# manhofer/Line3Dpp

Hardware: NVIDIA B200
Metric: matched_line_pairs_per_sec (higher is better)
Workload: dtype f32

## Files before the change

line3dpp_b200/csrc/l3d_match.cu:

```cuda
#include "l3d_match.cuh"
#include "l3d_device_f64.cuh"

__global__ void __launch_bounds__(256) k_prep_segments(const float4* __restrict__ segs, const L3DViewDev* __restrict__ views,
                                                       int num_views, long long total, float4* __restrict__ cache)
{
    long long idx = (long long)blockIdx.x * blockDim.x + threadIdx.x;
    if (idx >= total) return;
    int lo = 0, hi = num_views - 1;
    while (lo < hi) {
        int mid = (lo + hi + 1) >> 1;
        if (views[mid].seg_off <= idx) lo = mid; else hi = mid - 1;
    }
    const L3DViewDev* v = views + lo;
    float4 s = segs[idx];
    float3 r1 = normalize3(mulmat_h(v->RtKinv, s.x, s.y));
    float3 r2 = normalize3(mulmat_h(v->RtKinv, s.z, s.w));
    float3 n = normalize3(cross3(r1, r2));
    cache[3 * idx] = make_float4(r1.x, r1.y, r1.z, r2.x);
    cache[3 * idx + 1] = make_float4(r2.y, r2.z, n.x, n.y);
    cache[3 * idx + 2] = make_float4(n.z, 0.f, 0.f, 0.f);
}

__global__ void __launch_bounds__(256) k_prep_segments_f64(const float4* __restrict__ segs, const L3DViewDev* __restrict__ views,
                                                           int num_views, long long total, double* __restrict__ cache)
{
    long long idx = (long long)blockIdx.x * blockDim.x + threadIdx.x;
    if (idx >= total) return;
    int lo = 0, hi = num_views - 1;
    while (lo < hi) {
        int mid = (lo + hi + 1) >> 1;
        if (views[mid].seg_off <= idx) lo = mid; else hi = mid - 1;
    }
    const L3DViewDev* v = views + lo;
    float4 s = segs[idx];
    D3 r1 = dray(v->RtKinv_d, (double)s.x, (double)s.y), r2 = dray(v->RtKinv_d, (double)s.z, (double)s.w);
    D3 n = dnormalized(dcross(r1, r2));
    double* o = cache + 9 * idx;
    o[0] = r1.x; o[1] = r1.y; o[2] = r1.z; o[3] = r2.x; o[4] = r2.y; o[5] = r2.z; o[6] = n.x; o[7] = n.y; o[8] = n.z;
}

struct MatchSmem {
    uint4 stage[MK_STAGES][MK_TT];
    uint2 rowK[MK_ROWS];
    int cls_off[L3D_ARC_NCLS + 2];
    unsigned char rowall[MK_ROWS];
    unsigned long long lists[MK_ROWS][MK_CAP + 1];
    float4 rowA[MK_ROWS];
    float4 rowB[MK_ROWS];
    float row_thr[MK_ROWS];
    int list_cnt[MK_ROWS];
    unsigned int queue[MK_WARPS][128];
    unsigned int queue2[MK_WARPS][96];
    unsigned long long bars[MK_STAGES];
    const float4* tsegs; const float4* cache;
    long long src_base, toff;
    float3 Cs, Ct;
    float epi; int knn, Nt;
    int cap;
    const double* cache_d; const float4* ssegs;
    double Fd[9]; D3 Csd, Ctd;
    long long R0; l3d_match_rec* recs_out;
};
size_t l3d_match_smem_bytes() { return sizeof(MatchSmem); }

__device__ __forceinline__ int rank_in_row(const unsigned long long* list, int n, unsigned long long k)
{
    int r = 0;
    for (int j = 0; j < n; ++j) r += list[j] > k;
    return r;
}

__device__ __noinline__ void prune_row(MatchSmem& S, int row, int lane)
{
    const int knn = S.knn; const float epi = S.epi;
    __syncwarp();
    const int n = min(S.list_cnt[row], S.cap);
    const unsigned long long k = lane < n ? S.lists[row][lane] : 0ull;
    int r;
    if (knn <= 16) {
        bool active = lane < n;
        const unsigned int hi = (unsigned int)(k >> 32), lo = (unsigned int)k;
        r = 64;
        const int rounds = min(knn, n);
        for (int i = 0; i < rounds; ++i) {
            const unsigned int m = __reduce_max_sync(0xffffffffu, active ? hi : 0u);
            bool c = active && hi == m;
            unsigned int bm = __ballot_sync(0xffffffffu, c);
            if (__popc(bm) > 1) { const unsigned int l = __reduce_max_sync(0xffffffffu, c ? lo : 0u); c = c && lo == l; }
            if (c) { r = i; active = false; }
        }
    } else r = rank_in_row(S.lists[row], n, k);
    __syncwarp();
    if (lane < n && r < knn) S.lists[row][r] = k;
    __syncwarp();
    if (lane == 0) {
        S.list_cnt[row] = min(n, knn);
        if (n >= knn) {
            const float kth = key_overlap(S.lists[row][knn - 1]);
            S.row_thr[row] = kth;
            S.rowB[row].w = 0.95f * fmaxf(kth, epi);
        }
    }
    __syncwarp();
}

__device__ __noinline__ bool eval_candidate_f64(const MatchSmem& S, int rl, unsigned int j, float* ov_out, float* dep)
{
    const float4 sp = __ldg(S.ssegs + rl);
    const D3 e1 = dmulmat(S.Fd, d3((double)sp.x, (double)sp.y, 1.0)), e2 = dmulmat(S.Fd, d3((double)sp.z, (double)sp.w, 1.0));
    bool valid;
    const float ov = exact_overlap_f64(__ldg(S.tsegs + j), e1, e2, &valid);
    if (!(valid && ov > S.epi && ov >= S.row_thr[rl])) return false;
    const SegRaysD s = load_rays_d(S.cache_d, S.src_base + rl), t = load_rays_d(S.cache_d, S.toff + j);
    double d[4];
    exact_depths_f64(s, t, S.Csd, S.Ctd, d);
    if (!(d[0] > L3D_EPS_D && d[1] > L3D_EPS_D && d[2] > L3D_EPS_D && d[3] > L3D_EPS_D)) return false;
    *ov_out = ov;
    dep[0] = (float)d[0]; dep[1] = (float)d[1]; dep[2] = (float)d[2]; dep[3] = (float)d[3];
    return true;
}

template <int MODE, int KEEP>
__device__ __noinline__ void exact_batch(MatchSmem& S, unsigned int entry, bool has, int lane)
{
    const float4* __restrict__ tsegs = S.tsegs; const float4* __restrict__ cache = S.cache;
    const long long src_base = S.src_base, toff = S.toff;
    const float3 Cs = S.Cs, Ct = S.Ct;
    const float epi = S.epi; const int knn = S.knn;
    bool pending = false;
    unsigned long long key = 0ull;
    int rl = 0;
    if (has) {
        rl = (int)(entry >> 24);
        unsigned int j = entry & 0xFFFFFFu;
        if (j >= (unsigned int)S.Nt) j = 0u, has = false;
        float ov = 0.0f, d[4];
        bool ok = false;
        if (MODE) { if (has) ok = eval_candidate_f64(S, rl, j, &ov, d); }
        else {
            float4 q = __ldg(tsegs + j);
            float4 rA = S.rowA[rl], rB = S.rowB[rl];
            bool inv;
            ov = exact_overlap(q, make_float3(rA.x, rA.y, rA.z), make_float3(rA.w, rB.x, rB.y), &inv);
            if (has && ov > epi && ov >= S.row_thr[rl]) {
                SegRays s = load_rays(cache, src_base + rl), t = load_rays(cache, toff + j);
                exact_depths(s, t, Cs, Ct, d);
                ok = d[0] > 0.0f && d[1] > 0.0f && d[2] > 0.0f && d[3] > 0.0f;
            }
        }
        if (ok) {
            if (KEEP == 0) { key = make_key(ov, j); pending = true; }
            else {
                const int slot = atomicAdd(&S.list_cnt[rl], 1);
                if (KEEP == 2 && slot < knn) {
                    l3d_match_rec rec;
                    rec.tgt_seg = j; rec.overlap = ov; rec.d_p1 = d[0]; rec.d_p2 = d[1]; rec.d_q1 = d[2]; rec.d_q2 = d[3];
                    S.recs_out[(S.R0 + rl) * knn + slot] = rec;
                }
            }
        }
    }
    while (KEEP == 0) {
        if (pending) {
            int slot = atomicAdd(&S.list_cnt[rl], 1);
            if (slot < S.cap) { S.lists[rl][slot] = key; pending = false; }
        }
        unsigned int pm = __ballot_sync(0xffffffffu, pending);
        if (!pm) break;
        unsigned int todo = pm;
        while (todo) {
            int leader = __ffs(todo) - 1;
            int row = __shfl_sync(0xffffffffu, rl, leader);
            prune_row(S, row, lane);
            unsigned int mine = __ballot_sync(0xffffffffu, pending && rl == row);
            todo &= ~mine;
            if (knn >= S.cap) {
                while (mine) {
                    int l = __ffs(mine) - 1;
                    mine &= mine - 1;
                    unsigned long long k = __shfl_sync(0xffffffffu, key, l);
                    if (lane == 0 && k > S.lists[row][S.cap - 1]) S.lists[row][S.cap - 1] = k;
                    if (lane == l) pending = false;
                    prune_row(S, row, lane);
                }
            }
        }
    }
    __syncwarp();
}

template <int MODE, int KEEP>
__device__ __noinline__ void finalize_rows(MatchSmem& S, int warp, int lane, int nrows, long long R0, int* __restrict__ counts_out,
                                           l3d_match_rec* __restrict__ recs_out)
{
    const int knn = S.knn;
    for (int r = 0; r < MK_RPW; ++r) {
        const int rl = warp * MK_RPW + r;
        if (rl >= nrows) break;
        const long long R = R0 + rl;
        if (KEEP != 0) { if (lane == 0) counts_out[R] = S.list_cnt[rl]; continue; }
        const int n = min(S.list_cnt[rl], S.cap);
        if (lane == 0) counts_out[R] = min(n, knn);
        if (n == 0) continue;
        const unsigned long long key = lane < n ? S.lists[rl][lane] : 0ull;
        const int rank = rank_in_row(S.lists[rl], n, key);
        if (lane < n && rank < knn) {
            unsigned int j = key_tgt(key);
            float d[4];
            if (MODE) {
                const SegRaysD s = load_rays_d(S.cache_d, S.src_base + rl), t = load_rays_d(S.cache_d, S.toff + j);
                double dd[4];
                exact_depths_f64(s, t, S.Csd, S.Ctd, dd);
                d[0] = (float)dd[0]; d[1] = (float)dd[1]; d[2] = (float)dd[2]; d[3] = (float)dd[3];
            } else {
                SegRays s = load_rays(S.cache, S.src_base + rl), t = load_rays(S.cache, S.toff + j);
                exact_depths(s, t, S.Cs, S.Ct, d);
            }
            l3d_match_rec rec;
            rec.tgt_seg = j; rec.overlap = key_overlap(key);
            rec.d_p1 = d[0]; rec.d_p2 = d[1]; rec.d_q1 = d[2]; rec.d_q2 = d[3];
            recs_out[R * knn + rank] = rec;
        }
    }
}

__device__ void pair_basis(const float* F, L3DPairBasis* B)
{
    double c[3][3];
    for (int k = 0; k < 3; ++k) {
        const double x = F[k], y = F[3 + k], z = F[6 + k], n = sqrt(x * x + y * y + z * z);
        c[k][0] = n > 0.0 ? x / n : 0.0; c[k][1] = n > 0.0 ? y / n : 0.0; c[k][2] = n > 0.0 ? z / n : 0.0;
    }
    double E[3] = {0.0, 0.0, 0.0}, best = 0.0;
    for (int a = 0; a < 3; ++a)
        for (int b = a + 1; b < 3; ++b) {
            const double x = c[a][1] * c[b][2] - c[a][2] * c[b][1], y = c[a][2] * c[b][0] - c[a][0] * c[b][2], z = c[a][0] * c[b][1] - c[a][1] * c[b][0];
            const double n = x * x + y * y + z * z;
            if (n > best) { best = n; E[0] = x; E[1] = y; E[2] = z; }
        }
    const double nan = __longlong_as_double(0x7ff8000000000000ll);
    double n[3] = {E[0] / L3D_ARC_SCALE, E[1] / L3D_ARC_SCALE, E[2]};
    const double len = sqrt(n[0] * n[0] + n[1] * n[1] + n[2] * n[2]);
    if (!(best > 1e-20) || !(len > 0.0) || !isfinite(len)) { for (int i = 0; i < 3; ++i) B->u[i] = B->v[i] = nan; return; }
    for (int i = 0; i < 3; ++i) n[i] /= len;
    int ax = 0;
    if (fabs(n[1]) < fabs(n[ax])) ax = 1;
    if (fabs(n[2]) < fabs(n[ax])) ax = 2;
    double a[3] = {0.0, 0.0, 0.0}; a[ax] = 1.0;
    double u[3] = {n[1] * a[2] - n[2] * a[1], n[2] * a[0] - n[0] * a[2], n[0] * a[1] - n[1] * a[0]};
    const double ul = sqrt(u[0] * u[0] + u[1] * u[1] + u[2] * u[2]);
    for (int i = 0; i < 3; ++i) u[i] /= ul;
    const double v[3] = {n[1] * u[2] - n[2] * u[1], n[2] * u[0] - n[0] * u[2], n[0] * u[1] - n[1] * u[0]};
    for (int i = 0; i < 3; ++i) { B->u[i] = u[i]; B->v[i] = v[i]; }
}

__device__ uint4 target_arc(const L3DPairBasis& B, float4 q, double ext, bool enabled)
{
    const uint4 none = make_uint4(0u, 0xFFFFFFFFu, 0u, 0u);
    if (!enabled) return none;
    const double x1 = (double)q.x / L3D_ARC_SCALE, y1 = (double)q.y / L3D_ARC_SCALE, x2 = (double)q.z / L3D_ARC_SCALE, y2 = (double)q.w / L3D_ARC_SCALE;
    const double a1 = x1 * B.u[0] + y1 * B.u[1] + B.u[2], b1 = x1 * B.v[0] + y1 * B.v[1] + B.v[2];
    const double dx = x2 - x1, dy = y2 - y1, ac = dx * B.u[0] + dy * B.u[1], bc = dx * B.v[0] + dy * B.v[1];
    const double len = sqrt(dx * dx + dy * dy), rhoc = sqrt(ac * ac + bc * bc);
    const double delta = (0.05 + 4e-3 * len * L3D_ARC_SCALE) / L3D_ARC_SCALE;
    if (!(len > 1e-9) || !isfinite(rhoc) || !(rhoc > 1e-3 * len) || !(ext >= 0.0)) return none;
    {
        const double lx = y1 - y2, ly = x2 - x1, lz = x1 * y2 - y1 * x2;
        const double nx = B.u[1] * B.v[2] - B.u[2] * B.v[1], ny = B.u[2] * B.v[0] - B.u[0] * B.v[2], nz = B.u[0] * B.v[1] - B.u[1] * B.v[0];
        if (!(fabs(lx * nx + ly * ny + lz * nz) > 1e-4 * sqrt(lx * lx + ly * ly + lz * lz))) return none;
    }
    const double to_units = 4294967296.0 / 3.14159265358979323846;
    const unsigned int kc = arc_units(atan2(ac, -bc));
    const double ts[4] = {-ext, 0.0, 1.0, 1.0 + ext};
    double al[4], mg[4];
    for (int i = 0; i < 4; ++i) {
        const double a = a1 + ts[i] * ac, b = b1 + ts[i] * bc, rho = sqrt(a * a + b * b);
        if (!isfinite(rho) || !(delta < 0.25 * rho)) return none;
        al[i] = (double)(unsigned int)(arc_units(atan2(a, -b)) - kc);
        mg[i] = (1.2 * delta / rho + 4e-6) * to_units;
    }
    const bool up = al[0] <= al[1] && al[1] <= al[2] && al[2] <= al[3], down = al[0] >= al[1] && al[1] >= al[2] && al[2] >= al[3];
    if (!up && !down) return none;
    const int i0 = up ? 0 : 3, i1 = up ? 1 : 2, i2 = up ? 2 : 1, i3 = up ? 3 : 0;
    const double top = 4294967295.0;
    double lo = fmax(al[i1] - mg[i1], 0.0), hi = fmin(al[i2] + mg[i2], top);
    double lox = fmin(fmax(al[i0] - mg[i0], 0.0), lo), hix = fmax(fmin(al[i3] + mg[i3], top), hi);
    lo = floor(lo); lox = floor(lox); hi = ceil(hi); hix = ceil(hix);
    if (!(hix - lox < 2147483648.0 - 524288.0)) return none;
    return make_uint4(kc + (unsigned int)lo, (unsigned int)(hi - lo), (unsigned int)(lo - lox), (unsigned int)(hix - hi));
}

__global__ void __launch_bounds__(256)
k_pair_arcs(const float4* __restrict__ segs, const L3DViewDev* __restrict__ views, const L3DPairDev* __restrict__ pairs, int first_pair,
            int enabled, double ext, uint4* __restrict__ raw, unsigned long long* __restrict__ keys, unsigned int* __restrict__ vals,
            L3DPairBasis* __restrict__ basis)
{
    __shared__ L3DPairBasis B;
    __shared__ int cnt[L3D_ARC_NCLS + 1];
    const L3DPairDev* P = pairs + first_pair + blockIdx.x;
    if (threadIdx.x == 0) pair_basis(P->F, &B);
    if (threadIdx.x <= L3D_ARC_NCLS) cnt[threadIdx.x] = 0;
    __syncthreads();
    const L3DViewDev* vt = views + P->tgt;
    const float4* t = segs + vt->seg_off;
    const int Nt = vt->nseg;
    for (int j = threadIdx.x; j < Nt; j += 256) {
        const uint4 r = target_arc(B, t[j], ext, enabled != 0);
        const int c = arc_class(r.y);
        raw[P->arc_off + j] = r;
        keys[P->arc_off + j] = ((unsigned long long)blockIdx.x << 36) | ((unsigned long long)c << 32) | (c == L3D_ARC_NCLS ? (unsigned long long)j : (unsigned long long)r.x);
        vals[P->arc_off + j] = (unsigned int)(P->arc_off + j);
        atomicAdd(&cnt[c], 1);
    }
    __syncthreads();
    if (threadIdx.x == 0) {
        int off = 0;
        for (int c = 0; c <= L3D_ARC_NCLS; ++c) { B.cls_off[c] = off; off += cnt[c]; }
        B.cls_off[L3D_ARC_NCLS + 1] = off;
        basis[first_pair + blockIdx.x] = B;
    }
}

__global__ void __launch_bounds__(256)
k_arcs_gather(long long n, const unsigned long long* __restrict__ keys, const unsigned int* __restrict__ vals, const uint4* __restrict__ raw,
              const L3DPairDev* __restrict__ pairs, int first_pair, uint4* __restrict__ out)
{
    const long long i = (long long)blockIdx.x * blockDim.x + threadIdx.x;
    if (i >= n) return;
    const unsigned long long k = keys[i];
    const unsigned int src = vals[i];
    const uint4 r = raw[src];
    const bool wide = ((k >> 32) & 0xFull) == (unsigned long long)L3D_ARC_NCLS;
    const unsigned int j = src - (unsigned int)pairs[first_pair + (int)(k >> 36)].arc_off;
    const unsigned int w16 = (r.y + 65535u) >> 16, e1 = (r.z + 65535u) >> 16, eh = (r.w + 65535u) >> 16;
    out[i] = wide ? make_uint4(0u, 0u, L3D_ARC_WIDE, j) : make_uint4(r.x, e1 | (w16 << 16), eh, j);
}

template <int MODE, int KEEP>
__device__ __forceinline__ void filter_batch(MatchSmem& S, unsigned int e0, bool has0, unsigned int e1, bool has1, int warp, int lane,
                                             unsigned int lt_mask, int& qn2)
{
    float4 q0 = make_float4(0.f, 0.f, 0.f, 0.f), q1 = q0;
    if (has0) q0 = __ldg(S.tsegs + (e0 & 0xFFFFFFu));
    if (has1) q1 = __ldg(S.tsegs + (e1 & 0xFFFFFFu));
    bool p0 = false, p1 = false;
    if (has0) { const int rl = (int)(e0 >> 24); p0 = filter_may_survive(q0, S.rowA[rl], S.rowB[rl]); }
    if (has1) { const int rl = (int)(e1 >> 24); p1 = filter_may_survive(q1, S.rowA[rl], S.rowB[rl]); }
    const unsigned int b0 = __ballot_sync(0xffffffffu, p0), b1 = __ballot_sync(0xffffffffu, p1);
    if (b0 | b1) {
        if (p0) S.queue2[warp][qn2 + __popc(b0 & lt_mask)] = e0;
        qn2 += __popc(b0);
        if (p1) S.queue2[warp][qn2 + __popc(b1 & lt_mask)] = e1;
        qn2 += __popc(b1);
        __syncwarp();
        while (qn2 >= 32) { qn2 -= 32; exact_batch<MODE, KEEP>(S, S.queue2[warp][qn2 + lane], true, lane); }
    }
}

template <int MODE, int KEEP>
__device__ __forceinline__ void match_topk_body(const float4* __restrict__ segs, const float4* __restrict__ cache, const L3DViewDev* __restrict__ views,
             const L3DPairDev* __restrict__ pairs, const int2* __restrict__ tiles, int knn, float epi,
             int* __restrict__ counts_out, l3d_match_rec* __restrict__ recs_out, const double* __restrict__ cache_d,
             const uint4* __restrict__ arcs, const L3DPairBasis* __restrict__ basis)
{
    extern __shared__ __align__(128) unsigned char smem_raw[];
    MatchSmem& S = *reinterpret_cast<MatchSmem*>(smem_raw);
    const int tid = threadIdx.x, lane = tid & 31, warp = tid >> 5;
    const int2 tile = tiles[blockIdx.x];
    const L3DPairDev* P = pairs + tile.x;
    const int row0 = tile.y;
    const L3DViewDev* vs = views + P->src;
    const L3DViewDev* vt = views + P->tgt;
    const long long soff = vs->seg_off, toff = vt->seg_off;
    const int Ns = vs->nseg, Nt = vt->nseg;
    const int nrows = min(MK_ROWS, Ns - row0);
    const float4* tsegs = segs + toff;
    const uint4* tarcs = arcs + P->arc_off;
    const int RES = MK_STAGES * MK_TT;
    const int npass = (Nt + RES - 1) / RES;
    if (tid == 0) {
        S.tsegs = tsegs; S.cache = cache; S.src_base = soff + row0; S.toff = toff; S.epi = epi; S.knn = knn; S.Nt = Nt; S.cap = MK_CAP;
        S.Cs = make_float3(vs->C[0], vs->C[1], vs->C[2]); S.Ct = make_float3(vt->C[0], vt->C[1], vt->C[2]);
        S.cache_d = cache_d; S.ssegs = segs + soff + row0; S.R0 = P->row_off + row0; S.recs_out = recs_out;
        if (MODE) {
            for (int i = 0; i < 9; ++i) S.Fd[i] = P->Fd[i];
            S.Csd = d3(vs->C_d[0], vs->C_d[1], vs->C_d[2]); S.Ctd = d3(vt->C_d[0], vt->C_d[1], vt->C_d[2]);
        }
        for (int i = 0; i < MK_STAGES; ++i) mbar_init(&S.bars[i], 1);
        mbar_fence_init();
        for (int i = 0; i < MK_STAGES && i * MK_TT < Nt; ++i) {
            const unsigned int bytes = (unsigned int)min(MK_TT, Nt - i * MK_TT) * 16u;
            mbar_expect_tx(&S.bars[i], bytes);
            tma_load_1d(S.stage[i], tarcs + (size_t)i * MK_TT, bytes, &S.bars[i]);
        }
    }
    if (tid >= MK_THREADS - (L3D_ARC_NCLS + 2)) S.cls_off[MK_THREADS - 1 - tid] = basis[tile.x].cls_off[MK_THREADS - 1 - tid];
    if (tid < MK_ROWS) {
        S.list_cnt[tid] = 0;
        S.row_thr[tid] = 0.0f;
        if (tid < nrows) {
            float4 s = __ldg(segs + soff + row0 + tid);
            float3 e1 = mulmat_h(P->F, s.x, s.y), e2 = mulmat_h(P->F, s.z, s.w);
            float g = L3D_FILTER_C1 * fmaxf(sqrtf(e1.x * e1.x + e1.y * e1.y), sqrtf(e2.x * e2.x + e2.y * e2.y));
            S.rowA[tid] = make_float4(e1.x, e1.y, e1.z, e2.x);
            S.rowB[tid] = make_float4(e2.y, e2.z, g, 0.95f * epi);
            const L3DPairBasis B = basis[tile.x];
            bool off1, off2;
            S.rowK[tid] = make_uint2(line_kappa(B, e1, &off1), line_kappa(B, e2, &off2));
            S.rowall[tid] = (off1 || off2) ? 1 : 0;
        }
    }
    __syncthreads();

    const unsigned int lt_mask = (1u << lane) - 1u;
    const uint4* ent = &S.stage[0][0];
    const int my_rows = min(MK_RPW, nrows - warp * MK_RPW);
    int qn = 0, qn2 = 0;

    for (int pass = 0; pass < npass; ++pass) {
        const int base = pass * RES, cnt = min(RES, Nt - base);
        if (pass > 0) {
            __syncthreads();
            if (tid == 0)
                for (int i = 0; i < MK_STAGES && i * MK_TT < cnt; ++i) {
                    const unsigned int bytes = (unsigned int)min(MK_TT, cnt - i * MK_TT) * 16u;
                    mbar_expect_tx(&S.bars[i], bytes);
                    tma_load_1d(S.stage[i], tarcs + (size_t)base + (size_t)i * MK_TT, bytes, &S.bars[i]);
                }
        }
        for (int i = 0; i < MK_STAGES && i * MK_TT < cnt; ++i) mbar_wait(&S.bars[i], (unsigned int)(pass & 1));
        for (int r = 0; r < my_rows; ++r) {
            const int rl = warp * MK_RPW + r;
            const uint2 kr = S.rowK[rl];
            const bool rall = S.rowall[rl] != 0;
            const bool fwd = (kr.y - kr.x) < 0x80000000u;
            const unsigned int ka = fwd ? kr.x : kr.y, kb = fwd ? kr.y : kr.x;
            int res = 0;
            {
                const int c = min(lane >> 1, L3D_ARC_NCLS - 1);
                int lo = min(max(S.cls_off[c] - base, 0), cnt), hi = min(max(S.cls_off[c + 1] - base, 0), cnt);
                const bool upper = lane & 1;
                const unsigned int key = upper ? kb + 1u : ka - (1u << (L3D_ARC_CLS0 + c));
                if (lane >= 2 * L3D_ARC_NCLS || rall) hi = lo;
                else if (upper && kb == 0xFFFFFFFFu) lo = hi;
                while (lo < hi) {
                    const int mid = (lo + hi) >> 1;
                    if (ent[mid].x < key) lo = mid + 1; else hi = mid;
                }
                res = lo;
            }
            int plo = 0, phi = 0;
            {
                const int c = min(lane >> 1, L3D_ARC_NCLS - 1);
                const int i0 = __shfl_sync(0xffffffffu, res, 2 * c), i1 = __shfl_sync(0xffffffffu, res, 2 * c + 1);
                const int s_c = min(max(S.cls_off[c] - base, 0), cnt), e_c = min(max(S.cls_off[c + 1] - base, 0), cnt);
                const bool wrap = ka - (1u << (L3D_ARC_CLS0 + c)) > kb;
                if (lane < 2 * L3D_ARC_NCLS) {
                    if (!(lane & 1)) { plo = wrap ? s_c : i0; phi = i1; }
                    else if (wrap) { plo = i0; phi = e_c; }
                } else if (lane == 2 * L3D_ARC_NCLS) { plo = min(max(S.cls_off[L3D_ARC_NCLS] - base, 0), cnt); phi = cnt; }
                if (rall) { plo = 0; phi = lane == 0 ? cnt : 0; }
            }
            unsigned int pieces = __ballot_sync(0xffffffffu, phi > plo);
            while (pieces) {
                const int p = __ffs(pieces) - 1;
                pieces &= pieces - 1u;
                const int lo = __shfl_sync(0xffffffffu, plo, p), hi = __shfl_sync(0xffffffffu, phi, p);
                for (int j0 = lo; j0 < hi; j0 += 64) {
                    const int ia = j0 + lane, ib = ia + 32;
                    bool pa = false, pb = false;
                    unsigned int ta = 0u, tb = 0u;
                    if (ia < hi) { const uint4 e = ent[ia]; pa = arc_may_match(e, kr.x, kr.y) || rall; ta = e.w; }
                    if (ib < hi) { const uint4 e = ent[ib]; pb = arc_may_match(e, kr.x, kr.y) || rall; tb = e.w; }
                    const unsigned int ba = __ballot_sync(0xffffffffu, pa), bb = __ballot_sync(0xffffffffu, pb);
                    if (ba | bb) {
                        if (pa) S.queue[warp][qn + __popc(ba & lt_mask)] = ((unsigned int)rl << 24) | ta;
                        qn += __popc(ba);
                        if (pb) S.queue[warp][qn + __popc(bb & lt_mask)] = ((unsigned int)rl << 24) | tb;
                        qn += __popc(bb);
                        __syncwarp();
                        if (qn >= 64) {
                            qn -= 64;
                            filter_batch<MODE, KEEP>(S, S.queue[warp][qn + lane], true, S.queue[warp][qn + 32 + lane], true, warp, lane, lt_mask, qn2);
                        }
                    }
                }
            }
        }
    }
    if (qn > 0) {
        const bool h0 = lane < qn, h1 = lane + 32 < qn;
        filter_batch<MODE, KEEP>(S, h0 ? S.queue[warp][lane] : 0u, h0, h1 ? S.queue[warp][lane + 32] : 0u, h1, warp, lane, lt_mask, qn2);
    }
    __syncwarp();
    if (qn2 > 0) {
        const bool has = lane < qn2;
        exact_batch<MODE, KEEP>(S, has ? S.queue2[warp][lane] : 0u, has, lane);
    }
    __syncwarp();

    finalize_rows<MODE, KEEP>(S, warp, lane, nrows, P->row_off + row0, counts_out, recs_out);
}

__global__ void __launch_bounds__(MK_THREADS, MK_MINB)
k_match_topk(const float4* __restrict__ segs, const float4* __restrict__ cache, const L3DViewDev* __restrict__ views,
             const L3DPairDev* __restrict__ pairs, const int2* __restrict__ tiles, int knn, float epi,
             int* __restrict__ counts_out, l3d_match_rec* __restrict__ recs_out, const uint4* __restrict__ arcs, const L3DPairBasis* __restrict__ basis)
{ match_topk_body<0, 0>(segs, cache, views, pairs, tiles, knn, epi, counts_out, recs_out, nullptr, arcs, basis); }

__global__ void __launch_bounds__(MK_THREADS, MK_MINB)
k_match_topk_f64(const float4* __restrict__ segs, const float4* __restrict__ cache, const L3DViewDev* __restrict__ views,
                 const L3DPairDev* __restrict__ pairs, const int2* __restrict__ tiles, int knn, float epi,
                 int* __restrict__ counts_out, l3d_match_rec* __restrict__ recs_out, const double* __restrict__ cache_d,
                 const uint4* __restrict__ arcs, const L3DPairBasis* __restrict__ basis)
{ match_topk_body<1, 0>(segs, cache, views, pairs, tiles, knn, epi, counts_out, recs_out, cache_d, arcs, basis); }

__global__ void __launch_bounds__(MK_THREADS, MK_MINB)
k_match_all(const float4* __restrict__ segs, const float4* __restrict__ cache, const L3DViewDev* __restrict__ views,
            const L3DPairDev* __restrict__ pairs, const int2* __restrict__ tiles, int stride, float epi,
            int* __restrict__ counts_out, l3d_match_rec* __restrict__ recs_out, const double* __restrict__ cache_d,
            const uint4* __restrict__ arcs, const L3DPairBasis* __restrict__ basis)
{
    if (cache_d) {
        if (stride == 0) match_topk_body<1, 1>(segs, cache, views, pairs, tiles, 0, epi, counts_out, recs_out, cache_d, arcs, basis);
        else match_topk_body<1, 2>(segs, cache, views, pairs, tiles, stride, epi, counts_out, recs_out, cache_d, arcs, basis);
    } else {
        if (stride == 0) match_topk_body<0, 1>(segs, cache, views, pairs, tiles, 0, epi, counts_out, recs_out, nullptr, arcs, basis);
        else match_topk_body<0, 2>(segs, cache, views, pairs, tiles, stride, epi, counts_out, recs_out, nullptr, arcs, basis);
    }
}

__global__ void __launch_bounds__(128) k_sort_rows(int* __restrict__ counts, l3d_match_rec* __restrict__ recs, int stride, long long rows, int topk)
{
    extern __shared__ __align__(16) unsigned char sort_smem[];
    const int warp = threadIdx.x >> 5, lane = threadIdx.x & 31, wpb = blockDim.x >> 5;
    l3d_match_rec* buf = reinterpret_cast<l3d_match_rec*>(sort_smem) + (size_t)warp * stride;
    for (long long row = (long long)blockIdx.x * wpb + warp; row < rows; row += (long long)gridDim.x * wpb) {
        const int n = min(counts[row], stride);
        if (n > 1) {
            l3d_match_rec* g = recs + row * stride;
            for (int i = lane; i < n; i += 32) buf[i] = g[i];
            __syncwarp();
            for (int i = lane; i < n; i += 32) {
                const unsigned int t = buf[i].tgt_seg;
                const float ov = buf[i].overlap;
                int r = 0;
                if (topk > 0) { for (int j = 0; j < n; ++j) r += (buf[j].overlap > ov || (buf[j].overlap == ov && buf[j].tgt_seg < t)) ? 1 : 0; if (r < topk) g[r] = buf[i]; }
                else { for (int j = 0; j < n; ++j) r += buf[j].tgt_seg < t; g[r] = buf[i]; }
            }
        }
        if (topk > 0 && lane == 0 && n > topk) counts[row] = topk;
        __syncwarp();
    }
}

struct DenseSmem {
    float4 rowA[DK_ROWS], rowB[DK_ROWS];
    float4 sray[DK_ROWS][3];
    float4 tq[DK_WARPS][32 * DK_T];
    unsigned int queue[DK_WARPS][64];
    float4* depths; float* overlaps;
    const float4* tcache;
    float3 Cs, Ct;
    float epi; int Nt, row0;
};
size_t l3d_dense_smem_bytes() { return sizeof(DenseSmem); }
int l3d_dense_rows_per_cta(int Ns, int Nt, int num_sms)
{
    const long long slots = (long long)DK_MINB * (num_sms > 0 ? num_sms : 148);
    const long long colb = (Nt + DK_WARPS * DK_T * 32 - 1) / (DK_WARPS * DK_T * 32);
    int best = 16; double best_eff = -1.0;
    for (int R = 8; R <= DK_ROWS; ++R) {
        const long long tiles = colb * ((Ns + R - 1) / R);
        const long long waves = (tiles + slots - 1) / slots;
        const double eff = (double)tiles / (double)(waves * slots);
        if (eff > best_eff + 1e-9 || (eff > best_eff - 1e-9 && R > best)) { best_eff = eff; best = R; }
    }
    return best;
}

__device__ __forceinline__ SegRays rays_from_smem(const float4* p)
{
    const float4 a = p[0], b = p[1], c = p[2];
    SegRays s;
    s.r1 = make_float3(a.x, a.y, a.z); s.r2 = make_float3(a.w, b.x, b.y); s.n = make_float3(b.z, b.w, c.x);
    return s;
}

__device__ __noinline__ void dense_exact_batch(DenseSmem& S, unsigned int entry, bool has, int warp, int x0)
{
    if (!has) return;
    const int r = (int)(entry >> 24), x = (int)(entry & 0xFFFFFFu), col = x - x0;
    const float4 q = S.tq[warp][col];
    const float4 rA = S.rowA[r], rB = S.rowB[r];
    float4 res = make_float4(-1.f, -1.f, -1.f, -1.f);
    bool inv;
    const float ov = exact_overlap(q, make_float3(rA.x, rA.y, rA.z), make_float3(rA.w, rB.x, rB.y), &inv);
    if (ov > S.epi) {
        const SegRays s = rays_from_smem(S.sray[r]), t = load_rays(S.tcache, x);
        float d[4];
        exact_depths(s, t, S.Cs, S.Ct, d);
        res = make_float4(d[0], d[1], d[2], d[3]);
    }
    const size_t o = (size_t)(S.row0 + r) * S.Nt + x;
    __stcs(S.depths + o, res);
    __stcs(S.overlaps + o, ov);
}

__device__ __forceinline__ void dense_tile(const float4* __restrict__ ssegs, int Ns, const float4* __restrict__ tsegs, int Nt,
                                           const float4* __restrict__ scache, const float4* __restrict__ tcache, const L3DMat3& F, float3 Cs, float3 Ct,
                                           float epi, float4* __restrict__ depths, float* __restrict__ overlaps, int rows_per_cta, int bx, int by)
{
    extern __shared__ __align__(128) unsigned char dense_smem_raw[];
    DenseSmem& S = *reinterpret_cast<DenseSmem*>(dense_smem_raw);
    const int tid = threadIdx.x, lane = tid & 31, warp = tid >> 5;
    const int row0 = by * rows_per_cta;
    const int nrows = min(rows_per_cta, Ns - row0);
    if (tid == 0) { S.depths = depths; S.overlaps = overlaps; S.tcache = tcache; S.Cs = Cs; S.Ct = Ct; S.epi = epi; S.Nt = Nt; S.row0 = row0; }
    if (tid < nrows) {
        float4 s = __ldg(ssegs + row0 + tid);
        float3 e1 = mulmat_h(F.m, s.x, s.y), e2 = mulmat_h(F.m, s.z, s.w);
        float g = L3D_FILTER_C1 * fmaxf(sqrtf(e1.x * e1.x + e1.y * e1.y), sqrtf(e2.x * e2.x + e2.y * e2.y));
        S.rowA[tid] = make_float4(e1.x, e1.y, e1.z, e2.x);
        S.rowB[tid] = make_float4(e2.y, e2.z, g, 0.f);
    }
    if (tid < 3 * nrows) S.sray[tid / 3][tid % 3] = __ldg(scache + 3 * (size_t)row0 + tid);
    const int x0 = (bx * DK_WARPS + warp) * (32 * DK_T);
    float4 q[DK_T];
    bool ok[DK_T];
#pragma unroll
    for (int t = 0; t < DK_T; ++t) {
        const int x = x0 + t * 32 + lane;
        ok[t] = x < Nt;
        q[t] = __ldg(tsegs + (ok[t] ? x : 0));
        S.tq[warp][t * 32 + lane] = q[t];
    }
    __syncthreads();
    if (x0 >= Nt) return;
    const unsigned int lt_mask = (1u << lane) - 1u;
    const float4 none = make_float4(-1.f, -1.f, -1.f, -1.f);
    int qn = 0;
    for (int r = 0; r < nrows; ++r) {
        const float4 rA = S.rowA[r], rB = S.rowB[r];
        const size_t orow = (size_t)(row0 + r) * Nt;
        bool pass[DK_T];
#pragma unroll
        for (int t = 0; t < DK_T; ++t) pass[t] = ok[t] && filter_may_survive(q[t], rA, rB);
#pragma unroll
        for (int t = 0; t < DK_T; ++t) {
            const int x = x0 + t * 32 + lane;
            if (ok[t] && !pass[t]) { __stcs(depths + orow + x, none); __stcs(overlaps + orow + x, 0.0f); }
            const unsigned int b = __ballot_sync(0xffffffffu, pass[t]);
            if (b) {
                if (pass[t]) S.queue[warp][qn + __popc(b & lt_mask)] = ((unsigned int)r << 24) | (unsigned int)x;
                qn += __popc(b);
                __syncwarp();
                if (qn >= 32) { qn -= 32; dense_exact_batch(S, S.queue[warp][qn + lane], true, warp, x0); }
            }
        }
    }
    if (qn > 0) dense_exact_batch(S, lane < qn ? S.queue[warp][lane] : 0u, lane < qn, warp, x0);
}

__global__ void __launch_bounds__(DK_THREADS, DK_MINB)
k_match_dense(const float4* __restrict__ ssegs, int Ns, const float4* __restrict__ tsegs, int Nt,
              const float4* __restrict__ scache, const float4* __restrict__ tcache, L3DMat3 F, float3 Cs, float3 Ct,
              float epi, float4* __restrict__ depths, float* __restrict__ overlaps, int rows_per_cta)
{ dense_tile(ssegs, Ns, tsegs, Nt, scache, tcache, F, Cs, Ct, epi, depths, overlaps, rows_per_cta, blockIdx.x, blockIdx.y); }

__global__ void __launch_bounds__(DK_THREADS, DK_MINB)
k_match_dense_batch(const L3DDenseJob* __restrict__ jobs, int njobs, float epi)
{
    __shared__ int job_s;
    if (threadIdx.x == 0) {
        int lo = 0, hi = njobs - 1;
        while (lo < hi) { const int mid = (lo + hi + 1) >> 1; if (jobs[mid].tile0 <= (long long)blockIdx.x) lo = mid; else hi = mid - 1; }
        job_s = lo;
    }
    __syncthreads();
    const L3DDenseJob& J = jobs[job_s];
    const int t = (int)((long long)blockIdx.x - J.tile0);
    dense_tile(J.ssegs, J.Ns, J.tsegs, J.Nt, J.scache, J.tcache, J.F, J.Cs, J.Ct, epi, J.depths, J.overlaps, J.rows_per_cta, t % J.colb, t / J.colb);
}

__global__ void __launch_bounds__(DK_THREADS)
k_match_dense_nofilter(const float4* __restrict__ ssegs, int Ns, const float4* __restrict__ tsegs, int Nt,
                       const float4* __restrict__ scache, const float4* __restrict__ tcache, L3DMat3 F, float3 Cs,
                       float3 Ct, float epi, float4* __restrict__ depths, float* __restrict__ overlaps)
{
    const int x = blockIdx.x * DK_THREADS + threadIdx.x;
    const int row0 = blockIdx.y * DKN_ROWS;
    const int nrows = min(DKN_ROWS, Ns - row0);
    if (x >= Nt) return;
    const float4 q = __ldg(tsegs + x);
    for (int r = 0; r < nrows; ++r) {
        float4 s4 = __ldg(ssegs + row0 + r);
        float3 e1 = mulmat_h(F.m, s4.x, s4.y), e2 = mulmat_h(F.m, s4.z, s4.w);
        float4 res = make_float4(-1.f, -1.f, -1.f, -1.f);
        bool inv;
        float ov = exact_overlap(q, e1, e2, &inv);
        if (ov > epi) {
            SegRays s = load_rays(scache, row0 + r), t = load_rays(tcache, x);
            float d[4];
            exact_depths(s, t, Cs, Ct, d);
            res = make_float4(d[0], d[1], d[2], d[3]);
        }
        const size_t o = (size_t)(row0 + r) * Nt + x;
        depths[o] = res;
        overlaps[o] = ov;
    }
}

__global__ void __launch_bounds__(256) k_compact_matches(const int* __restrict__ counts, const long long* __restrict__ row_ptr,
                                                         const l3d_match_rec* __restrict__ recs, int knn, long long rows,
                                                         l3d_match_rec* __restrict__ out)
{
    long long i = (long long)blockIdx.x * blockDim.x + threadIdx.x;
    long long row = i / knn;
    int slot = (int)(i - row * knn);
    if (row >= rows) return;
    if (slot < counts[row]) out[row_ptr[row] + slot] = recs[row * knn + slot];
}

__global__ void __launch_bounds__(256) k_fp32_peak(float* __restrict__ out, int iters, float a, float b)
{
    float x[16];
#pragma unroll
    for (int i = 0; i < 16; ++i) x[i] = (float)(threadIdx.x + i);
    for (int it = 0; it < iters; ++it) {
#pragma unroll
        for (int i = 0; i < 16; ++i) x[i] = __fmaf_rn(x[i], a, b);
    }
    float s = 0.f;
#pragma unroll
    for (int i = 0; i < 16; ++i) s += x[i];
    if (s == 123.456f) out[0] = s;
}
```

line3dpp_b200/csrc/l3d_match.cuh:

```cuda
#pragma once
#include "l3d_device.cuh"
#include "../../include/l3d_capi.h"

#ifndef MK_WARPS
#define MK_WARPS 8
#endif
#define MK_THREADS (32 * MK_WARPS)
#ifndef MK_RPW
#define MK_RPW 8
#endif
#define MK_ROWS (MK_WARPS * MK_RPW)
#ifndef MK_TT
#define MK_TT 1024
#endif
#ifndef MK_STAGES
#define MK_STAGES 3
#endif
#ifndef MK_CAP
#define MK_CAP 32
#endif
#ifndef MK_MINB
#define MK_MINB 3
#endif

#define DK_THREADS 256
#ifndef DK_MINB
#define DK_MINB 4
#endif
#define DK_WARPS 8
#define DK_ROWS 32
#define DK_T 4
#define DKN_ROWS 32

struct L3DMat3 { float m[9]; };

size_t l3d_match_smem_bytes();
size_t l3d_dense_smem_bytes();

__global__ void k_prep_segments(const float4* __restrict__ segs, const L3DViewDev* __restrict__ views, int num_views,
                                long long total, float4* __restrict__ cache);
__global__ void k_match_topk(const float4* __restrict__ segs, const float4* __restrict__ cache,
                             const L3DViewDev* __restrict__ views, const L3DPairDev* __restrict__ pairs,
                             const int2* __restrict__ tiles, int knn, float epi, int* __restrict__ counts_out,
                             l3d_match_rec* __restrict__ recs_out, const uint4* __restrict__ arcs, const L3DPairBasis* __restrict__ basis);
__global__ void k_match_topk_f64(const float4* __restrict__ segs, const float4* __restrict__ cache,
                                 const L3DViewDev* __restrict__ views, const L3DPairDev* __restrict__ pairs,
                                 const int2* __restrict__ tiles, int knn, float epi, int* __restrict__ counts_out,
                                 l3d_match_rec* __restrict__ recs_out, const double* __restrict__ cache_d, const uint4* __restrict__ arcs,
                                 const L3DPairBasis* __restrict__ basis);
__global__ void k_match_all(const float4* __restrict__ segs, const float4* __restrict__ cache,
                            const L3DViewDev* __restrict__ views, const L3DPairDev* __restrict__ pairs,
                            const int2* __restrict__ tiles, int stride, float epi, int* __restrict__ counts_out,
                            l3d_match_rec* __restrict__ recs_out, const double* __restrict__ cache_d, const uint4* __restrict__ arcs,
                            const L3DPairBasis* __restrict__ basis);
__global__ void k_pair_arcs(const float4* __restrict__ segs, const L3DViewDev* __restrict__ views, const L3DPairDev* __restrict__ pairs,
                            int first_pair, int enabled, double ext, uint4* __restrict__ raw, unsigned long long* __restrict__ keys,
                            unsigned int* __restrict__ vals, L3DPairBasis* __restrict__ basis);
__global__ void k_arcs_gather(long long n, const unsigned long long* __restrict__ keys, const unsigned int* __restrict__ vals,
                              const uint4* __restrict__ raw, const L3DPairDev* __restrict__ pairs, int first_pair, uint4* __restrict__ out);
__global__ void k_sort_rows(int* __restrict__ counts, l3d_match_rec* __restrict__ recs, int stride, long long rows, int topk);
__global__ void k_prep_segments_f64(const float4* __restrict__ segs, const L3DViewDev* __restrict__ views, int num_views,
                                    long long total, double* __restrict__ cache);
__global__ void k_match_dense(const float4* __restrict__ ssegs, int Ns, const float4* __restrict__ tsegs, int Nt,
                              const float4* __restrict__ scache, const float4* __restrict__ tcache, L3DMat3 F, float3 Cs,
                              float3 Ct, float epi, float4* __restrict__ depths, float* __restrict__ overlaps, int rows_per_cta);
int l3d_dense_rows_per_cta(int Ns, int Nt, int num_sms);
struct L3DDenseJob {
    const float4* ssegs; const float4* tsegs; const float4* scache; const float4* tcache; float4* depths; float* overlaps;
    L3DMat3 F; float3 Cs, Ct; int Ns, Nt, rows_per_cta, colb; long long tile0;
};
__global__ void k_match_dense_batch(const L3DDenseJob* __restrict__ jobs, int njobs, float epi);
__global__ void k_match_dense_nofilter(const float4* __restrict__ ssegs, int Ns, const float4* __restrict__ tsegs, int Nt,
                                       const float4* __restrict__ scache, const float4* __restrict__ tcache, L3DMat3 F,
                                       float3 Cs, float3 Ct, float epi, float4* __restrict__ depths,
                                       float* __restrict__ overlaps);
__global__ void k_compact_matches(const int* __restrict__ counts, const long long* __restrict__ row_ptr,
                                  const l3d_match_rec* __restrict__ recs, int knn, long long rows,
                                  l3d_match_rec* __restrict__ out);
__global__ void k_fp32_peak(float* __restrict__ out, int iters, float a, float b);
```

Before: 481.1 billion.

## Replace append-then-prune top-k lists with warp-resident sorted insertion

Each row's top-k list becomes a sorted array of up to 32 keys kept in warp registers. New candidates are inserted with shuffle-up and ballot, replacing the old append buffer and its periodic prune_row rank/reduce passes. This removes the separate prune step, the cap handling and the final rank computation in output, since lists are already sorted by lane. It adds zero-initialisation of the lists in shared memory and assumes knn is at most 32. It also adds an optional compile-time counter of exact evaluations.

```diff
diff --git a/line3dpp_b200/csrc/l3d_match.cu b/line3dpp_b200/csrc/l3d_match.cu
--- a/line3dpp_b200/csrc/l3d_match.cu
+++ b/line3dpp_b200/csrc/l3d_match.cu
@@ -44,7 +44,7 @@
     uint2 rowK[MK_ROWS];
     int cls_off[L3D_ARC_NCLS + 2];
     unsigned char rowall[MK_ROWS];
-    unsigned long long lists[MK_ROWS][MK_CAP + 1];
+    unsigned long long lists[MK_ROWS][32];
     float4 rowA[MK_ROWS];
     float4 rowB[MK_ROWS];
     float row_thr[MK_ROWS];
@@ -56,53 +56,24 @@
     long long src_base, toff;
     float3 Cs, Ct;
     float epi; int knn, Nt;
-    int cap;
     const double* cache_d; const float4* ssegs;
     double Fd[9]; D3 Csd, Ctd;
     long long R0; l3d_match_rec* recs_out;
 };
 size_t l3d_match_smem_bytes() { return sizeof(MatchSmem); }
 
-__device__ __forceinline__ int rank_in_row(const unsigned long long* list, int n, unsigned long long k)
-{
-    int r = 0;
-    for (int j = 0; j < n; ++j) r += list[j] > k;
-    return r;
-}
-
-__device__ __noinline__ void prune_row(MatchSmem& S, int row, int lane)
-{
-    const int knn = S.knn; const float epi = S.epi;
-    __syncwarp();
-    const int n = min(S.list_cnt[row], S.cap);
-    const unsigned long long k = lane < n ? S.lists[row][lane] : 0ull;
-    int r;
-    if (knn <= 16) {
-        bool active = lane < n;
-        const unsigned int hi = (unsigned int)(k >> 32), lo = (unsigned int)k;
-        r = 64;
-        const int rounds = min(knn, n);
-        for (int i = 0; i < rounds; ++i) {
-            const unsigned int m = __reduce_max_sync(0xffffffffu, active ? hi : 0u);
-            bool c = active && hi == m;
-            unsigned int bm = __ballot_sync(0xffffffffu, c);
-            if (__popc(bm) > 1) { const unsigned int l = __reduce_max_sync(0xffffffffu, c ? lo : 0u); c = c && lo == l; }
-            if (c) { r = i; active = false; }
-        }
-    } else r = rank_in_row(S.lists[row], n, k);
-    __syncwarp();
-    if (lane < n && r < knn) S.lists[row][r] = k;
-    __syncwarp();
-    if (lane == 0) {
-        S.list_cnt[row] = min(n, knn);
-        if (n >= knn) {
-            const float kth = key_overlap(S.lists[row][knn - 1]);
-            S.row_thr[row] = kth;
-            S.rowB[row].w = 0.95f * fmaxf(kth, epi);
-        }
-    }
-    __syncwarp();
-}
+#ifdef L3D_COUNT_EXACT
+__device__ unsigned long long l3d_exact_evals;
+extern "C" unsigned long long l3d_exact_evals_take()
+{
+    unsigned long long n = 0ull;
+    const unsigned long long zero = 0ull;
+    cudaDeviceSynchronize();
+    cudaMemcpyFromSymbol(&n, l3d_exact_evals, sizeof(n));
+    cudaMemcpyToSymbol(l3d_exact_evals, &zero, sizeof(zero));
+    return n;
+}
+#endif
 
 __device__ __noinline__ bool eval_candidate_f64(const MatchSmem& S, int rl, unsigned int j, float* ov_out, float* dep)
 {
@@ -130,6 +101,9 @@
     bool pending = false;
     unsigned long long key = 0ull;
     int rl = 0;
+#ifdef L3D_COUNT_EXACT
+    { const unsigned int n = __popc(__ballot_sync(0xffffffffu, has)); if (lane == 0 && n) atomicAdd(&l3d_exact_evals, (unsigned long long)n); }
+#endif
     if (has) {
         rl = (int)(entry >> 24);
         unsigned int j = entry & 0xFFFFFFu;
@@ -160,30 +134,26 @@
             }
         }
     }
-    while (KEEP == 0) {
-        if (pending) {
-            int slot = atomicAdd(&S.list_cnt[rl], 1);
-            if (slot < S.cap) { S.lists[rl][slot] = key; pending = false; }
-        }
-        unsigned int pm = __ballot_sync(0xffffffffu, pending);
-        if (!pm) break;
-        unsigned int todo = pm;
+    unsigned int pm = KEEP == 0 ? __ballot_sync(0xffffffffu, pending) : 0u;
+    while (pm) {
+        const int row = __shfl_sync(0xffffffffu, rl, __ffs(pm) - 1);
+        unsigned int todo = __ballot_sync(0xffffffffu, pending && rl == row);
+        pm &= ~todo;
+        unsigned long long mine = lane < knn ? S.lists[row][lane] : 0ull;
         while (todo) {
-            int leader = __ffs(todo) - 1;
-            int row = __shfl_sync(0xffffffffu, rl, leader);
-            prune_row(S, row, lane);
-            unsigned int mine = __ballot_sync(0xffffffffu, pending && rl == row);
-            todo &= ~mine;
-            if (knn >= S.cap) {
-                while (mine) {
-                    int l = __ffs(mine) - 1;
-                    mine &= mine - 1;
-                    unsigned long long k = __shfl_sync(0xffffffffu, key, l);
-                    if (lane == 0 && k > S.lists[row][S.cap - 1]) S.lists[row][S.cap - 1] = k;
-                    if (lane == l) pending = false;
-                    prune_row(S, row, lane);
-                }
-            }
+            const int l = __ffs(todo) - 1;
+            todo &= todo - 1u;
+            const unsigned long long k = __shfl_sync(0xffffffffu, key, l);
+            const unsigned long long up = __shfl_up_sync(0xffffffffu, mine, 1);
+            const bool below = lane < knn && mine < k;
+            const unsigned int bl = __ballot_sync(0xffffffffu, below);
+            if (below) mine = lane == __ffs(bl) - 1 ? k : up;
+        }
+        if (lane < knn) S.lists[row][lane] = mine;
+        const unsigned long long kth = __shfl_sync(0xffffffffu, mine, knn - 1);
+        if (lane == 0 && kth != 0ull) {
+            S.row_thr[row] = key_overlap(kth);
+            S.rowB[row].w = 0.95f * fmaxf(key_overlap(kth), epi);
         }
     }
     __syncwarp();
@@ -199,12 +169,10 @@
         if (rl >= nrows) break;
         const long long R = R0 + rl;
         if (KEEP != 0) { if (lane == 0) counts_out[R] = S.list_cnt[rl]; continue; }
-        const int n = min(S.list_cnt[rl], S.cap);
-        if (lane == 0) counts_out[R] = min(n, knn);
-        if (n == 0) continue;
-        const unsigned long long key = lane < n ? S.lists[rl][lane] : 0ull;
-        const int rank = rank_in_row(S.lists[rl], n, key);
-        if (lane < n && rank < knn) {
+        const unsigned long long key = lane < knn ? S.lists[rl][lane] : 0ull;
+        const unsigned int have = __ballot_sync(0xffffffffu, key != 0ull);
+        if (lane == 0) counts_out[R] = __popc(have);
+        if (key != 0ull) {
             unsigned int j = key_tgt(key);
             float d[4];
             if (MODE) {
@@ -219,7 +187,7 @@
             l3d_match_rec rec;
             rec.tgt_seg = j; rec.overlap = key_overlap(key);
             rec.d_p1 = d[0]; rec.d_p2 = d[1]; rec.d_q1 = d[2]; rec.d_q2 = d[3];
-            recs_out[R * knn + rank] = rec;
+            recs_out[R * knn + lane] = rec;
         }
     }
 }
@@ -379,7 +347,7 @@
     const int RES = MK_STAGES * MK_TT;
     const int npass = (Nt + RES - 1) / RES;
     if (tid == 0) {
-        S.tsegs = tsegs; S.cache = cache; S.src_base = soff + row0; S.toff = toff; S.epi = epi; S.knn = knn; S.Nt = Nt; S.cap = MK_CAP;
+        S.tsegs = tsegs; S.cache = cache; S.src_base = soff + row0; S.toff = toff; S.epi = epi; S.knn = knn; S.Nt = Nt;
         S.Cs = make_float3(vs->C[0], vs->C[1], vs->C[2]); S.Ct = make_float3(vt->C[0], vt->C[1], vt->C[2]);
         S.cache_d = cache_d; S.ssegs = segs + soff + row0; S.R0 = P->row_off + row0; S.recs_out = recs_out;
         if (MODE) {
@@ -395,6 +363,7 @@
         }
     }
     if (tid >= MK_THREADS - (L3D_ARC_NCLS + 2)) S.cls_off[MK_THREADS - 1 - tid] = basis[tile.x].cls_off[MK_THREADS - 1 - tid];
+    for (int i = tid; i < MK_ROWS * 32; i += MK_THREADS) S.lists[i >> 5][i & 31] = 0ull;
     if (tid < MK_ROWS) {
         S.list_cnt[tid] = 0;
         S.row_thr[tid] = 0.0f;
diff --git a/line3dpp_b200/csrc/l3d_match.cuh b/line3dpp_b200/csrc/l3d_match.cuh
--- a/line3dpp_b200/csrc/l3d_match.cuh
+++ b/line3dpp_b200/csrc/l3d_match.cuh
@@ -15,9 +15,6 @@
 #endif
 #ifndef MK_STAGES
 #define MK_STAGES 3
-#endif
-#ifndef MK_CAP
-#define MK_CAP 32
 #endif
 #ifndef MK_MINB
 #define MK_MINB 3
```

Result: slower. 475.5 billion (median of 6 runs) (-1.2%).
